# Penguin-jpg/clip-diffusion

Measured on NVIDIA B200. Metric: CLIP-guided cutouts/s fwd+bwd inside full guidance steps (= steps/s x cutouts per step) @512x512, higher is better.
Workload: dtype bf16

## Files before the change

clip_diffusion_b200/csrc/vit_attention_tc.cu:

```cuda
#include "common.cuh"
#include "tcgen05.cuh"

using namespace tc;

namespace {

constexpr int AT_THREADS = 512;
constexpr int MAX_BLK = 5;
static_assert((ATTN_TC_MAX_T + 63) / 64 <= MAX_BLK, "operand blocks of the longest sequence");
constexpr float LOG2E_F = 1.4426950408889634f;
constexpr uint32_t BLK_BYTES = 64 * 128;
constexpr uint32_t TILE_BYTES = 128 * 128;

__device__ __forceinline__ uint32_t pack_bf2(float a, float b) {
  __nv_bfloat162 v = __floats2bfloat162_rn(a, b);
  return *reinterpret_cast<uint32_t*>(&v);
}
__device__ __forceinline__ float ex2f(float x) {
  float y;
  asm("ex2.approx.ftz.f32 %0, %1;" : "=f"(y) : "f"(x));
  return y;
}
__device__ __forceinline__ float warp_max_f(float v) {
#pragma unroll
// ... 586 lines not shown
                w[j] = pack_bf2(p0, p1);
              }
            }
            lsum += a0 + a1;
            TRF(warp, g, 5 + hlf);
            if (!waited) { mbar_wait(bars.pfree(b), (use & 1u) ^ 1u); waited = true; }
            const uint32_t hb = sStage + b * TILE_BYTES + (uint32_t)rl * 128u;
            st_shared_v4(hb + (((uint32_t)(hlf * 64)) ^ sx), w[0], w[1], w[2], w[3]);
            st_shared_v4(hb + (((uint32_t)(hlf * 64 + 16)) ^ sx), w[4], w[5], w[6], w[7]);
            st_shared_v4(hb + (((uint32_t)(hlf * 64 + 32)) ^ sx), w[8], w[9], w[10], w[11]);
            st_shared_v4(hb + (((uint32_t)(hlf * 64 + 48)) ^ sx), w[12], w[13], w[14], w[15]);
          }
        }
        if (last_in_tile) {
          const int tp = tile & 1, a = 2 * wg + tp;
          const uint32_t u = tp ? wuse1 : wuse0;
          if (wvalid) {
            sm[(a * 4 + (int)(u & 3u)) * 128 + rl] = mref;
            sl[(a * 4 + (int)(u & 3u)) * 128 + rl] = lsum;
          }
          __syncwarp();
          if (lane == 0) mbar_arrive(bars.mready(a, u & 1u));
          if (tp) wuse1 = u + 1; else wuse0 = u + 1;
        }
        TRF(warp, g, 2);
        fence_proxy_async_smem();
        __syncwarp();
        if (lane == 0) mbar_arrive(bars.pready(b));
        TRF(warp, g, 3);
        blk += 2;
        while (blk >= nblk) { blk -= nblk; ++tile; }
      }
    }
  } else {
    const int q = warp & 3;
    const int rl = q * 32 + lane;
    const uint32_t t_lane = tmem_base + ((uint32_t)(q * 32) << 16);
    const float sl2 = p.scale * LOG2E_F;
    float* vedge2 = pvec + 808;
    uint32_t euse = 0;
    auto edge_a = [&](int wi, int eit, float& s0, float& s1) {
      const uint32_t opar = (uint32_t)eit & 1u;
      if (edge) {
        for (int b = 0; b < nblk_ld; ++b) { mbar_wait(bars.opk(b), opar); mbar_wait(bars.opq(b), opar); }
#ifdef CG_ATTN_TRACE
        long long* etr = (p.trace != nullptr && blockIdx.x == 0 && eit == 3) ? p.trace + ((warp * 64 + 60) << 3) : nullptr;
#else
        long long* etr = nullptr;
#endif
        const float2 se = fwd_edge_token_a(sQ, sK, Tp, sl2, pvec, etr);
        s0 = se.x;
        s1 = se.y;
      } else if (eit > 0) {
        mbar_wait(bars.qkfree(), (uint32_t)(eit - 1) & 1u);
      }
      __syncwarp();
      if (lane == 0) mbar_arrive(bars.qkfree());
    };
    auto edge_b = [&](int wi, int eit) {
      const int n = wi / heads, h = wi - n * heads, row0 = n * T, vb = eit & 1;
      if (edge) {
        for (int b = 0; b < nblk_ld; ++b) mbar_wait(bars.opv(vb, b), (uint32_t)(eit >> 1) & 1u);
#ifdef CG_ATTN_TRACE
        long long* etr = (p.trace != nullptr && blockIdx.x == 0 && eit == 3) ? p.trace + ((warp * 64 + 60) << 3) : nullptr;
#else
        long long* etr = nullptr;
#endif
        fwd_edge_token_b(sV0 + vb * opb, Tp, pvec, vedge2 + vb * 64, p.ctx + ((long long)(row0 + Tp)) * D + h * 64, p.lse + ((long long)n * heads + h) * T + Tp, etr);
      }
      __syncwarp();
      if (lane == 0) mbar_arrive(bars.vfree(vb));
    };
    float se0 = -INFINITY, se1 = -INFINITY, nse0 = -INFINITY, nse1 = -INFINITY;
    if ((int)blockIdx.x < nitems) { edge_a(blockIdx.x, 0, se0, se1); edge_b(blockIdx.x, 0); }
    int it = 0, gg0 = 0;
    for (int w = blockIdx.x; w < nitems; w += gridDim.x, ++it, gg0 += G) {
      const int n = w / heads, h = w - n * heads, row0 = n * T;
      const float* vedge = vedge2 + (it & 1) * 64;
      TRF(warp, 62, 0);
      TRI(warp, 0);
      for (int tile = 0; tile < ntiles; ++tile) {
        const int tp = tile & 1, a0 = tp, a1 = 2 + tp;
        const int ggt = gg0 + tile * nblk;
        const bool has0 = nblk > 1 || (ggt & 1) == 0, has1 = nblk > 1 || (ggt & 1) == 1;
        const uint32_t u0 = (euse >> (4 * a0)) & 15u, u1 = (euse >> (4 * a1)) & 15u;
        if (has0) { mbar_wait(bars.mready(a0, u0 & 1u), (u0 >> 1) & 1u); mbar_wait(bars.accfull(a0), u0 & 1u); }
        if (has1) { mbar_wait(bars.mready(a1, u1 & 1u), (u1 >> 1) & 1u); mbar_wait(bars.accfull(a1), u1 & 1u); }
        TRF(warp, tile, 0);
        tcgen05_fence_after();
        const int row = tile * 128 + rl;
        if (tile * 128 + q * 32 < Tp) {
          const float m0 = has0 ? sm[(a0 * 4 + (int)(u0 & 3u)) * 128 + rl] : -INFINITY, m1 = has1 ? sm[(a1 * 4 + (int)(u1 & 3u)) * 128 + rl] : -INFINITY;
          const float l0 = has0 ? sl[(a0 * 4 + (int)(u0 & 3u)) * 128 + rl] : 0.f, l1 = has1 ? sl[(a1 * 4 + (int)(u1 & 3u)) * 128 + rl] : 0.f;
          const float se = tile == 0 ? se0 : se1;
          const float M = fmaxf(fmaxf(m0, m1), se);
          const float f0 = has0 ? ex2f(m0 - M) : 0.f, f1 = has1 ? ex2f(m1 - M) : 0.f, fe = ex2f(se - M);
          const float L = l0 * f0 + l1 * f1 + fe;
          const float invL = __fdividef(1.f, L);
          const float g0 = f0 * invL, g1 = f1 * invL, ge = fe * invL;
          __nv_bfloat16* dst = p.ctx + ((long long)(row0 + row)) * D + h * 64;
#pragma unroll
          for (int c = 0; c < 64; c += 32) {
            uint32_t v0[32], v1[32], wv[16];
            if (has0) tmem_ld32(t_lane + 256u + (uint32_t)(a0 * 64 + c), v0);
            if (has1) tmem_ld32(t_lane + 256u + (uint32_t)(a1 * 64 + c), v1);
            tmem_ld_wait();
#pragma unroll
            for (int j = 0; j < 16; ++j) {
              float x0 = (has0 ? __uint_as_float(v0[2 * j]) * g0 : 0.f) + (has1 ? __uint_as_float(v1[2 * j]) * g1 : 0.f);
              float x1 = (has0 ? __uint_as_float(v0[2 * j + 1]) * g0 : 0.f) + (has1 ? __uint_as_float(v1[2 * j + 1]) * g1 : 0.f);
              if (edge) {
                const float2 ve = *reinterpret_cast<const float2*>(vedge + c + 2 * j);
                x0 = fmaf(ge, ve.x, x0);
                x1 = fmaf(ge, ve.y, x1);
              }
              wv[j] = pack_bf2(x0, x1);
            }
            if (row < Tp) { st256g(dst + c, wv); st256g(dst + c + 16, wv + 8); }
          }
          if (row < Tp) p.lse[((long long)n * heads + h) * T + row] = M * (1.f / LOG2E_F) + logf(L);
        }
        tcgen05_fence_before();
        __syncwarp();
        if (lane == 0) {
          if (has0) mbar_arrive(bars.accfree(a0));
          if (has1) mbar_arrive(bars.accfree(a1));
        }
        if (has0) euse = (euse & ~(15u << (4 * a0))) | (((u0 + 1u) & 15u) << (4 * a0));
        if (has1) euse = (euse & ~(15u << (4 * a1))) | (((u1 + 1u) & 15u) << (4 * a1));
        TRF(warp, tile, 1);
        if (tile == 0 && w + (int)gridDim.x < nitems) {
          TRF(warp, 61, 0);
          edge_a(w + gridDim.x, it + 1, nse0, nse1);
          edge_b(w + gridDim.x, it + 1);
          TRF(warp, 61, 1);
        }
      }
      se0 = nse0;
      se1 = nse1;
      TRF(warp, 62, 1);
      TRI(warp, 1);
    }
  }
  tcgen05_fence_before();
  __syncthreads();
  if (warp == 2) {
    tcgen05_fence_after();
    asm volatile("tcgen05.dealloc.cta_group::1.sync.aligned.b32 %0, %1;" ::"r"(tmem_base), "r"(512) : "memory");
  }
}

struct BBars {
  uint32_t base;
  __device__ __forceinline__ uint32_t sfull(int b) const { return base + 8u * b; }
  __device__ __forceinline__ uint32_t sfree(int b) const { return base + 24u + 8u * b; }
  __device__ __forceinline__ uint32_t pready(int pb) const { return base + 48u + 8u * pb; }
  __device__ __forceinline__ uint32_t pfree(int pb) const { return base + 64u + 8u * pb; }
  __device__ __forceinline__ uint32_t accfull(int a) const { return base + 80u + 8u * a; }
  __device__ __forceinline__ uint32_t accfree(int a) const { return base + 104u + 8u * a; }
  __device__ __forceinline__ uint32_t op(int o, int blk) const { return base + 128u + 8u * (o * MAX_BLK + blk); }
  __device__ __forceinline__ uint32_t opfree() const { return base + 288u; }
  __device__ __forceinline__ uint32_t cready(int par) const { return base + 296u + 8u * par; }
  __device__ __forceinline__ uint32_t tmem_slot() const { return base + 312u; }
};
constexpr uint32_t BBARS_BYTES = 320 + 16;
constexpr uint32_t BWD_FLOATS = 1280 + 1152 + 192 + 768;

#ifdef CG_ATTN_TRACE
#define TRB(slot, idx, ev) TRF(slot, idx, ev)
#else
#define TRB(slot, idx, ev) do { } while (0)
#endif

__device__ __forceinline__ void store_row64_bf16_axpy(__nv_bfloat16* dst, const uint32_t* a, const uint32_t* b, float coef, const float* vec) {
  uint32_t w[32];
#pragma unroll
  for (int j = 0; j < 16; ++j) {
    const float2 v0 = *reinterpret_cast<const float2*>(vec + 2 * j), v1 = *reinterpret_cast<const float2*>(vec + 32 + 2 * j);
    w[j] = pack_bf2(fmaf(coef, v0.x, __uint_as_float(a[2 * j])), fmaf(coef, v0.y, __uint_as_float(a[2 * j + 1])));
    w[16 + j] = pack_bf2(fmaf(coef, v1.x, __uint_as_float(b[2 * j])), fmaf(coef, v1.y, __uint_as_float(b[2 * j + 1])));
  }
#pragma unroll
  for (int j = 0; j < 4; ++j) st256g(dst + 16 * j, w + 8 * j);
}

__global__ void __launch_bounds__(AT_THREADS, 1)
    attn_bwd_tc_kernel(const __grid_constant__ CUtensorMap tmQKV, const __grid_constant__ CUtensorMap tmQKVtail, const __grid_constant__ CUtensorMap tmDO,
                       const __grid_constant__ CUtensorMap tmDOtail, const AttnParams p) {
  extern __shared__ __align__(1024) uint8_t smem_raw[];
  cg_griddep_launch();
  constexpr int NSB = 3;
  constexpr uint32_t STAGE_BYTES = 2 * TILE_BYTES;
  const int T = p.T, heads = p.heads, D = heads * 64;
  const int edge = p.edge, Tp = T - edge;
  const int warp = threadIdx.x >> 5, lane = threadIdx.x & 31;
  const int ntiles = p.ntiles, nblk = p.nblk, nblk_ld = p.nblk_ld;
  const int per_phase = ntiles * nblk, G = 2 * per_phase, nitems = p.nitems;
  const uint32_t opb = (uint32_t)((nblk_ld - 1) * 64 + p.ld_tail) * 128u;
  const uint32_t base = (smem_u32(smem_raw) + 1023u) & ~1023u;
  const uint32_t sOp0 = base;
  const uint32_t sStage = base + 4 * opb;
  const uint32_t sF = sStage + 2 * STAGE_BYTES;
  float* fscr = reinterpret_cast<float*>(smem_raw + (sF - smem_u32(smem_raw)));
  float* csts = fscr;
  float* ev = fscr + 1280;
  float* evec = fscr + 2432;
  float* epart = fscr + 2624;
  BBars bars{sF + BWD_FLOATS * 4};

  if (warp == 0 && lane == 0) {
    asm volatile("prefetch.tensormap [%0];" ::"l"(&tmQKV) : "memory");
    asm volatile("prefetch.tensormap [%0];" ::"l"(&tmQKVtail) : "memory");
    asm volatile("prefetch.tensormap [%0];" ::"l"(&tmDO) : "memory");
    asm volatile("prefetch.tensormap [%0];" ::"l"(&tmDOtail) : "memory");
    for (int b = 0; b < 3; ++b) {
      mbar_init(bars.sfull(b), 2); mbar_init(bars.sfree(b), 4);
      mbar_init(bars.accfull(b), 2); mbar_init(bars.accfree(b), 4);
    }
    for (int b = 0; b < 2; ++b) { mbar_init(bars.pready(b), 4); mbar_init(bars.pfree(b), 2); mbar_init(bars.cready(b), 4); }
    for (int o = 0; o < 4; ++o)
      for (int k = 0; k < MAX_BLK; ++k) mbar_init(bars.op(o, k), 1);
    mbar_init(bars.opfree(), 8);
    asm volatile("fence.mbarrier_init.release.cluster;" ::: "memory");
  }
  if (warp == 2) {
    asm volatile("tcgen05.alloc.cta_group::1.sync.aligned.shared::cta.b32 [%0], %1;" ::"r"(bars.tmem_slot()), "r"(512) : "memory");
    asm volatile("tcgen05.relinquish_alloc_permit.cta_group::1.sync.aligned;" ::: "memory");
  }
  cg_griddep_wait();
  tcgen05_fence_before();
  __syncthreads();
  tcgen05_fence_after();
  uint32_t tmem_base;
  asm volatile("ld.shared.b32 %0, [%1];" : "=r"(tmem_base) : "r"(bars.tmem_slot()) : "memory");

  if (warp < 4) {
    const uint32_t elected = elect_one();
    const uint32_t id_full = idesc_bf16(64, false), id_tail = idesc_bf16(p.tail_rows, false), id_acc = idesc_bf16(64, true);
    uint32_t cuse = 0;
    int it = 0, gg0 = 0;
    for (int w = blockIdx.x; w < nitems; w += gridDim.x, ++it, gg0 += G) {
      const uint32_t opar = (uint32_t)it & 1u;
      uint32_t loaded = 0;
      auto need = [&](int o, int blk) {
        const uint32_t bit = 1u << (o * MAX_BLK + blk);
        if (!(loaded & bit)) { mbar_wait(bars.op(o, blk), opar); loaded |= bit; }
      };
      if (warp == 3) {
        if (elected) {
          if (it > 0) mbar_wait(bars.opfree(), (uint32_t)(it - 1) & 1u);
          const int n = w / heads, h = w - n * heads, row0 = n * T;
          auto load = [&](int o, int blk) {
            const bool tail = blk == nblk_ld - 1;
            const uint32_t bar = bars.op(o, blk);
            mbar_arrive_expect_tx(bar, (uint32_t)(tail ? p.ld_tail : 64) * 128u);
            if (o < 3) tma_load_2d(sOp0 + o * opb + blk * BLK_BYTES, tail ? &tmQKVtail : &tmQKV, bar, o * D + h * 64, row0 + blk * 64);
            else tma_load_2d(sOp0 + o * opb + blk * BLK_BYTES, tail ? &tmDOtail : &tmDO, bar, h * 64, row0 + blk * 64);
          };
          const int first = nblk_ld < 2 ? nblk_ld : 2;
          load(1, 0);
#pragma unroll 1
          for (int k = 0; k < first; ++k) load(0, k);
          load(2, 0);
#pragma unroll 1
          for (int k = 0; k < first; ++k) load(3, k);
#pragma unroll 1
          for (int k = 1; k < nblk_ld; ++k) { load(1, k); load(2, k); }
#pragma unroll 1
          for (int k = first; k < nblk_ld; ++k) { load(0, k); load(3, k); }
          if (w + (int)gridDim.x < nitems) {
            const int w2 = w + gridDim.x, n2 = w2 / heads, h2 = w2 - n2 * heads;
#pragma unroll 1
            for (int k = 0; k < nblk_ld; ++k) {
              const bool tail = k == nblk_ld - 1;
#pragma unroll 1
              for (int o = 0; o < 3; ++o) tma_prefetch_2d(tail ? &tmQKVtail : &tmQKV, o * D + h2 * 64, n2 * T + k * 64);
              tma_prefetch_2d(tail ? &tmDOtail : &tmDO, h2 * 64, n2 * T + k * 64);
            }
          }
        }
        __syncwarp();
      }
      int phase = 0, tile = 0, blk = 0;
      if (warp < 2) {
        for (int g = 0; g < G; ++g) {
          const int gg = gg0 + g, b = gg % NSB;
          const bool transposed = phase == 1;
          const int oa = warp == 0 ? (transposed ? 1 : 0) : (transposed ? 2 : 3);
          const int ob = warp == 0 ? (transposed ? 0 : 1) : (transposed ? 3 : 2);
          need(oa, 2 * tile);
          if (2 * tile + 1 < nblk) need(oa, 2 * tile + 1);
          need(ob, blk);
          mbar_wait(bars.sfree(b), ((uint32_t)(gg / NSB) & 1u) ^ 1u);
          TRB(warp, g, 0);
          tcgen05_fence_after();
          const uint32_t d_s = tmem_base + (uint32_t)(b * 128) + (warp == 1 ? 64u : 0u);
          const uint64_t ad = make_smem_desc(sOp0 + oa * opb + tile * TILE_BYTES), bd = make_smem_desc(sOp0 + ob * opb + blk * BLK_BYTES);
          const uint32_t idesc = blk == nblk - 1 ? id_tail : id_full;
          if (elected) {
#pragma unroll
            for (int k = 0; k < 4; ++k) umma_bf16(d_s, ad + (uint64_t)(2 * k), bd + (uint64_t)(2 * k), idesc, k != 0 ? 1u : 0u);
            umma_commit(bars.sfull(b));
          }
          __syncwarp();
          TRB(warp, g, 1);
          if (++blk == nblk) { blk = 0; if (++tile == ntiles) { tile = 0; ++phase; } }
        }
      } else {
        const int wi = warp - 2;
        for (int g = 0; g < G; ++g) {
          const int gg = gg0 + g, pb = gg & 1;
          const int a = phase == 1 ? 2 : (tile & 1);
          const bool does_mma = phase == 1 || wi == 0;
          const int ob = phase == 0 ? 1 : (wi == 0 ? 3 : 0);
          if (does_mma) need(ob, blk);
          mbar_wait(bars.pready(pb), (uint32_t)(gg >> 1) & 1u);
          TRB(warp, g, 0);
          if (blk == 0) {
            if (phase == 1) {
              mbar_wait(bars.accfree(2), ((cuse >> 2) & 1u) ^ 1u);
              if (tile == 0) { mbar_wait(bars.accfree(0), (cuse & 1u) ^ 1u); mbar_wait(bars.accfree(1), ((cuse >> 1) & 1u) ^ 1u); }
            } else {
              mbar_wait(bars.accfree(a), ((cuse >> a) & 1u) ^ 1u);
              mbar_wait(bars.accfree(2), ((cuse >> 2) & 1u) ^ 1u);
            }
          }
          tcgen05_fence_after();
          const int ksteps = (blk == nblk - 1 ? p.tail_rows : 64) >> 4;
          const uint32_t stage = sStage + pb * STAGE_BYTES + (wi == 1 ? TILE_BYTES : 0u);
          const uint32_t d_acc = tmem_base + (a == 2 ? 384u : 384u + 64u * a) + (wi == 1 ? 64u : 0u);
          const uint64_t ad = make_smem_desc(stage), bd = make_smem_desc(sOp0 + ob * opb + blk * BLK_BYTES);
          const bool last = blk == nblk - 1;
          if (elected) {
            if (does_mma) {
              for (int k = 0; k < ksteps; ++k) umma_bf16(d_acc, ad + (uint64_t)(2 * k), bd + (uint64_t)(128 * k), id_acc, (blk | k) != 0 ? 1u : 0u);
              umma_commit(bars.pfree(pb));
              if (last) umma_commit(bars.accfull(a));
            } else {
              mbar_arrive(bars.pfree(pb));
              if (last) mbar_arrive(bars.accfull(a));
            }
          }
          __syncwarp();
          TRB(warp, g, 1);
          if (last) cuse ^= 1u << a;
          if (++blk == nblk) { blk = 0; if (++tile == ntiles) { tile = 0; ++phase; } }
        }
      }
#pragma unroll 1
      for (int o = 0; o < 4; ++o)
#pragma unroll 1
        for (int k = 0; k < nblk_ld; ++k) need(o, k);
      if (elected) umma_commit(bars.opfree());
      __syncwarp();
    }
  } else if (warp < 12) {
    const int wg = (warp - 4) >> 2;
    const int q = warp & 3;
    const int rl = q * 32 + lane;
    const uint32_t t_lane = tmem_base + ((uint32_t)(q * 32) << 16);
    const float scale = p.scale, sl2 = p.scale * LOG2E_F;
    const int tail_cols = Tp - (nblk - 1) * 64, tail_cols16 = p.tail_rows;
    const uint32_t sx = (uint32_t)(rl & 7) << 4;
    int it = 0, gg0 = 0;
    for (int w = blockIdx.x; w < nitems; w += gridDim.x, ++it, gg0 += G) {
      mbar_wait(bars.cready(it & 1), (uint32_t)(it >> 1) & 1u);
      const float* cst = csts + (it & 1) * 640;
      float rc0 = 0.f, rc1 = 0.f;
      int phase = 0, tile = 0, blk = wg, cur_tile = -1;
      while (blk >= nblk) { blk -= nblk; if (++tile == ntiles) { tile = 0; ++phase; } }
      for (int g = wg; g < G; g += 2) {
        const int gg = gg0 + g;
        if (phase == 0 && tile != cur_tile) {
          const int row = tile * 128 + rl;
          rc0 = row < Tp ? cst[row] : 0.f;
          rc1 = row < Tp ? cst[320 + row] : 0.f;
          cur_tile = tile;
        }
        const bool wvalid = tile * 128 + q * 32 < Tp;
        const bool tail = blk == nblk - 1;
        const int ncols = tail ? tail_cols : 64, ncols16 = tail ? tail_cols16 : 64;
        const int b = gg % NSB, pb = gg & 1;
        const uint32_t suse = (uint32_t)(gg / NSB), puse = (uint32_t)(gg >> 1);
        TRB(warp, g, 0);
        mbar_wait(bars.sfull(b), suse & 1u);
        TRB(warp, g, 1);
        tcgen05_fence_after();
        const uint32_t t_s = t_lane + (uint32_t)(b * 128);
        const uint32_t stage = sStage + pb * STAGE_BYTES + (uint32_t)rl * 128u;
        if (!wvalid) {
          tcgen05_fence_before();
          __syncwarp();
          if (lane == 0) mbar_arrive(bars.sfree(b));
          mbar_wait(bars.pfree(pb), (puse & 1u) ^ 1u);
        } else {
          uint32_t sv[2][16], dv[2][16], w0[8], w1[8];
          const int npieces = ncols16 >> 4;
          tmem_ld16(t_s, sv[0]);
          tmem_ld16(t_s + 64u, dv[0]);
          tmem_ld_wait();
          bool waited = false;
#pragma unroll
          for (int pc = 0; pc < 4; ++pc) {
            if (pc < npieces) {
              const int cur = pc & 1;
              if (pc + 1 < npieces) {
                tmem_ld16(t_s + (uint32_t)(16 * (pc + 1)), sv[cur ^ 1]);
                tmem_ld16(t_s + 64u + (uint32_t)(16 * (pc + 1)), dv[cur ^ 1]);
              }
              if (phase == 0) {
#pragma unroll
                for (int j = 0; j < 8; ++j) {
                  float p0 = ex2f(fmaf(__uint_as_float(sv[cur][2 * j]), sl2, rc0)), p1 = ex2f(fmaf(__uint_as_float(sv[cur][2 * j + 1]), sl2, rc0));
                  if (tail) { if (16 * pc + 2 * j >= ncols) p0 = 0.f; if (16 * pc + 2 * j + 1 >= ncols) p1 = 0.f; }
                  w0[j] = pack_bf2(p0 * fmaf(__uint_as_float(dv[cur][2 * j]), scale, rc1), p1 * fmaf(__uint_as_float(dv[cur][2 * j + 1]), scale, rc1));
                }
              } else {
                const float* nl = cst + blk * 64 + 16 * pc;
                const float* dl = nl + 320;
#pragma unroll
                for (int j = 0; j < 8; ++j) {
                  const float2 l2 = *reinterpret_cast<const float2*>(nl + 2 * j), d2 = *reinterpret_cast<const float2*>(dl + 2 * j);
                  float p0 = ex2f(fmaf(__uint_as_float(sv[cur][2 * j]), sl2, l2.x)), p1 = ex2f(fmaf(__uint_as_float(sv[cur][2 * j + 1]), sl2, l2.y));
                  if (tail) { if (16 * pc + 2 * j >= ncols) p0 = 0.f; if (16 * pc + 2 * j + 1 >= ncols) p1 = 0.f; }
                  w0[j] = pack_bf2(p0, p1);
                  w1[j] = pack_bf2(p0 * fmaf(__uint_as_float(dv[cur][2 * j]), scale, d2.x), p1 * fmaf(__uint_as_float(dv[cur][2 * j + 1]), scale, d2.y));
                }
              }
              if (!waited) { mbar_wait(bars.pfree(pb), (puse & 1u) ^ 1u); waited = true; }
              {
                const uint32_t c0 = ((uint32_t)(pc * 32)) ^ sx, c1 = ((uint32_t)(pc * 32 + 16)) ^ sx;
                st_shared_v4(stage + c0, w0[0], w0[1], w0[2], w0[3]);
                st_shared_v4(stage + c1, w0[4], w0[5], w0[6], w0[7]);
                if (phase == 1) {
                  st_shared_v4(stage + TILE_BYTES + c0, w1[0], w1[1], w1[2], w1[3]);
                  st_shared_v4(stage + TILE_BYTES + c1, w1[4], w1[5], w1[6], w1[7]);
                }
              }
              if (pc + 1 < npieces) {
                tmem_ld_wait();
              } else {
                tcgen05_fence_before();
                __syncwarp();
                if (lane == 0) mbar_arrive(bars.sfree(b));
              }
            }
          }
        }
        TRB(warp, g, 2);
        fence_proxy_async_smem();
        __syncwarp();
        if (lane == 0) mbar_arrive(bars.pready(pb));
        TRB(warp, g, 3);
        blk += 2;
        while (blk >= nblk) { blk -= nblk; if (++tile == ntiles) { tile = 0; ++phase; } }
      }
    }
  } else {
    const int q = warp & 3;
    const int rl = q * 32 + lane;
    const uint32_t t_lane = tmem_base + ((uint32_t)(q * 32) << 16);
    const float scale = p.scale, sl2 = p.scale * LOG2E_F;
    uint32_t euse = 0;
    auto load_consts = [&](int item, int par) {
      const int n = item / heads, h = item - n * heads;
      const float* lb = p.lse + ((long long)n * heads + h) * T;
      const __nv_bfloat16* ob = p.ctx_in + ((long long)n * T) * D + h * 64;
      const __nv_bfloat16* gb = p.dctx_in + ((long long)n * T) * D + h * 64;
      float* c = csts + par * 640;
      for (int i = rl; i < 320; i += 128) {
        float dl = 0.f, nl = -INFINITY;
        if (i < T) {
          const uint4* o4 = reinterpret_cast<const uint4*>(ob + (long long)i * D);
          const uint4* g4 = reinterpret_cast<const uint4*>(gb + (long long)i * D);
          uint4 xo[8], xg[8];
#pragma unroll
          for (int k = 0; k < 8; ++k) { xo[k] = __ldg(o4 + k); xg[k] = __ldg(g4 + k); }
          float d0 = 0.f, d1 = 0.f;
#pragma unroll
          for (int k = 0; k < 8; k += 2) { d0 = dot8p(xo[k], xg[k], d0); d1 = dot8p(xo[k + 1], xg[k + 1], d1); }
          dl = d0 + d1;
          nl = -lb[i] * LOG2E_F;
        }
        c[i] = nl;
        c[320 + i] = -p.scale * dl;
      }
      __syncwarp();
      if (lane == 0) mbar_arrive(bars.cready(par));
    };
    if ((int)blockIdx.x < nitems) load_consts(blockIdx.x, 0);
    int it = 0;
    for (int w = blockIdx.x; w < nitems; w += gridDim.x, ++it) {
      const int n = w / heads, h = w - n * heads, row0 = n * T;
      const uint32_t opar = (uint32_t)it & 1u;
      if (w + (int)gridDim.x < nitems) load_consts(w + gridDim.x, (it + 1) & 1);
      const float* cst = csts + (it & 1) * 640;
      __nv_bfloat16* out = p.dqkv + ((long long)row0) * 3 * D + h * 64;
      TRB(warp, 62, 0);
      TRI(warp, 0);
      if (edge) {
        for (int o = 0; o < 4; ++o)
          for (int k = 0; k < nblk_ld; ++k) mbar_wait(bars.op(o, k), opar);
        mbar_wait(bars.cready(it & 1), (uint32_t)(it >> 1) & 1u);
        TRB(warp, 61, 0);
        const uint32_t sQ = sOp0, sK = sOp0 + opb, sV = sOp0 + 2 * opb, sDO = sOp0 + 3 * opb;
        const float nle = cst[Tp], dle = cst[320 + Tp];
        const int g = lane >> 2, t = lane & 3;
        {
          uint32_t vbk[8], vbv[8], vbq[8], vbd[8];
          load_vec_bfrag(sK, Tp, vbk);
          load_vec_bfrag(sV, Tp, vbv);
          load_vec_bfrag(sQ, Tp, vbq);
          load_vec_bfrag(sDO, Tp, vbd);
#pragma unroll 1
          for (int rg = q; rg < (Tp >> 4); rg += 4) {
            const float2 s_c = mv16(sQ, rg * 16, vbk), dp_c = mv16(sDO, rg * 16, vbv), s_r = mv16(sK, rg * 16, vbq), dp_r = mv16(sV, rg * 16, vbd);
            if (t == 0) {
#pragma unroll
              for (int hh = 0; hh < 2; ++hh) {
                const int i = rg * 16 + g + 8 * hh;
                const float p_c = ex2f(fmaf(hh ? s_c.y : s_c.x, sl2, cst[i]));
                ev[i] = p_c;
                ev[288 + i] = p_c * fmaf(hh ? dp_c.y : dp_c.x, scale, cst[320 + i]);
                const float p_r = ex2f(fmaf(hh ? s_r.y : s_r.x, sl2, nle));
                ev[576 + i] = p_r;
                ev[864 + i] = p_r * fmaf(hh ? dp_r.y : dp_r.x, scale, dle);
              }
            }
          }
        }
        {
          const uint32_t eo = (uint32_t)Tp * 128u + (uint32_t)lane * 4u;
          const uint32_t wq = lds32(sQ + eo), wk = lds32(sK + eo), wv = lds32(sV + eo), wd = lds32(sDO + eo);
          const float s_e = warp_sum(fmaf(bf_lo(wq), bf_lo(wk), bf_hi(wq) * bf_hi(wk)));
          const float dp_e = warp_sum(fmaf(bf_lo(wd), bf_lo(wv), bf_hi(wd) * bf_hi(wv)));
          const float p_e = ex2f(fmaf(s_e, sl2, nle)), ds_e = p_e * fmaf(dp_e, scale, dle);
          if (rl == 0) { ev[Tp] = p_e; ev[288 + Tp] = ds_e; ev[576 + Tp] = p_e; ev[864 + Tp] = ds_e; }
          if (rl >= 1 && rl < 16) { ev[Tp + rl] = 0.f; ev[288 + Tp + rl] = 0.f; ev[576 + Tp + rl] = 0.f; ev[864 + Tp + rl] = 0.f; }
          if (q == 0) {
            evec[2 * lane] = bf_lo(wk); evec[2 * lane + 1] = bf_hi(wk);
            evec[64 + 2 * lane] = bf_lo(wq); evec[64 + 2 * lane + 1] = bf_hi(wq);
            evec[128 + 2 * lane] = bf_lo(wd); evec[128 + 2 * lane + 1] = bf_hi(wd);
          }
        }
        asm volatile("bar.sync 2, 128;" ::: "memory");
        {
          const int ngrp = (Tp >> 4) + 1;
#pragma unroll 1
          for (int pr = 0; pr < 3; ++pr) {
            const uint32_t buf = pr == 0 ? sK : (pr == 1 ? sQ : sDO);
            const float* vec = ev + (pr == 0 ? 864 : (pr == 1 ? 288 : 0));
            float acc[8][4];
#pragma unroll
            for (int nn = 0; nn < 8; ++nn) acc[nn][0] = acc[nn][1] = acc[nn][2] = acc[nn][3] = 0.f;
#pragma unroll 1
            for (int ks = q; ks < ngrp; ks += 4) vm16(buf, ks * 16, vec, acc);
            if (lane < 4) {
#pragma unroll
              for (int nn = 0; nn < 8; ++nn) *reinterpret_cast<float2*>(epart + (pr * 4 + q) * 64 + 8 * nn + 2 * t) = make_float2(acc[nn][0], acc[nn][1]);
            }
          }
          asm volatile("bar.sync 2, 128;" ::: "memory");
          if (q < 3) {
            const float* pp = epart + q * 256 + 2 * lane;
            const float2 x0 = *reinterpret_cast<const float2*>(pp), x1 = *reinterpret_cast<const float2*>(pp + 64);
            const float2 x2 = *reinterpret_cast<const float2*>(pp + 128), x3 = *reinterpret_cast<const float2*>(pp + 192);
            reinterpret_cast<uint32_t*>(out + (long long)Tp * 3 * D + q * D)[lane] = pack_bf2((x0.x + x1.x) + (x2.x + x3.x), (x0.y + x1.y) + (x2.y + x3.y));
          }
        }
        TRB(warp, 61, 1);
      }
      __syncwarp();
      if (lane == 0) mbar_arrive(bars.opfree());
      for (int tc = 0; tc < 2 * ntiles; ++tc) {
        const int phase = tc >= ntiles ? 1 : 0, tile = tc - phase * ntiles;
        const int a = phase == 1 ? 2 : (tile & 1);
        const int row = tile * 128 + rl;
        mbar_wait(bars.accfull(a), (euse >> a) & 1u);
        TRB(warp, tc, 0);
        tcgen05_fence_after();
        if (tile * 128 + q * 32 < Tp) {
          uint32_t v0[32], v1[32];
          const uint32_t col = a == 2 ? 384u : 384u + 64u * a;
          tmem_ld32(t_lane + col, v0);
          tmem_ld32(t_lane + col + 32u, v1);
          tmem_ld_wait();
          __nv_bfloat16* orow = out + (long long)row * 3 * D;
          if (phase == 0) {
            if (row < Tp) {
              if (edge) store_row64_bf16_axpy(orow, v0, v1, ev[288 + row], evec);
              else store_row64_bf16(orow, v0, v1, 1.f);
            }
          } else {
            if (row < Tp) {
              if (edge) store_row64_bf16_axpy(orow + 2 * D, v0, v1, ev[576 + row], evec + 128);
              else store_row64_bf16(orow + 2 * D, v0, v1, 1.f);
            }
            tmem_ld32(t_lane + col + 64u, v0);
            tmem_ld32(t_lane + col + 96u, v1);
            tmem_ld_wait();
            if (row < Tp) {
              if (edge) store_row64_bf16_axpy(orow + D, v0, v1, ev[864 + row], evec + 64);
              else store_row64_bf16(orow + D, v0, v1, 1.f);
            }
          }
        }
        tcgen05_fence_before();
        __syncwarp();
        if (lane == 0) mbar_arrive(bars.accfree(a));
        euse ^= 1u << a;
        TRB(warp, tc, 1);
      }
      TRB(warp, 62, 1);
      TRI(warp, 1);
    }
  }
  tcgen05_fence_before();
  __syncthreads();
  if (warp == 2) {
    tcgen05_fence_after();
    asm volatile("tcgen05.dealloc.cta_group::1.sync.aligned.b32 %0, %1;" ::"r"(tmem_base), "r"(512) : "memory");
  }
}

long long* g_trace = nullptr;

void set_geometry(AttnParams& p, int T, int heads, bool causal) {
  p.T = T; p.heads = heads; p.scale = 0.125f;
  p.trace = g_trace;
  p.edge = (!causal && T > 1 && (T - 1) % 64 == 0) ? 1 : 0;
  const int Tp = T - p.edge;
  p.ntiles = (Tp + 127) / 128;
  p.nblk = (Tp + 63) / 64;
  p.tail_rows = ((Tp - (p.nblk - 1) * 64) + 15) & ~15;
  p.nblk_ld = p.nblk + p.edge;
  p.ld_tail = p.edge ? 16 : p.tail_rows;
}

int make_operand_maps(CUtensorMap& full, CUtensorMap& tail, const void* ptr, long long rows, long long cols, const AttnParams& p) {
  const int rc = cg_make_tensor_map_bf16(&full, ptr, rows, cols, cols, 64);
  return rc ? rc : cg_make_tensor_map_bf16(&tail, ptr, rows, cols, cols, p.ld_tail);
}

template <auto kernel, typename... Maps>
int launch_persistent(AttnParams& p, int Nimg, size_t extra, cudaStream_t s, const Maps&... maps) {
  const size_t opb = (size_t)((p.nblk_ld - 1) * 64 + p.ld_tail) * 128;
  const size_t smem = 1024 + 4 * opb + 4 * (size_t)TILE_BYTES + extra;
  p.nitems = Nimg * p.heads;
  const int grid = p.nitems < cg_num_sms() ? p.nitems : cg_num_sms();
  static size_t configured[CG_MAX_DEVICES] = {};
  const int dev = cg_device_index();
  if (smem > configured[dev]) {
    CG_CUDA(cudaFuncSetAttribute(kernel, cudaFuncAttributeMaxDynamicSharedMemorySize, (int)smem));
    configured[dev] = smem;
  }
  CG_CUDA(cg_launch_pdl(kernel, dim3(grid), dim3(AT_THREADS), smem, s, maps..., p));
  return 0;
}

template <bool CAUSAL>
int launch_attn_fwd_tc(const void* qkv, int Nimg, int T, int heads, void* ctx, float* lse, cudaStream_t s) {
  AttnParams p = {};
  p.ctx = reinterpret_cast<__nv_bfloat16*>(ctx);
  p.lse = lse;
  set_geometry(p, T, heads, CAUSAL);
  CUtensorMap tq, tqt;
  const int rc = make_operand_maps(tq, tqt, qkv, (long long)Nimg * T, 3LL * heads * 64, p);
  if (rc) return rc;
  return launch_persistent<attn_fwd_tc_kernel<CAUSAL>>(p, Nimg, FWD_FLOATS * 4 + FBARS_BYTES, s, tq, tqt);
}

}

int cg_attention_fwd_tc(const void* qkv, int Nimg, int T, int heads, void* ctx, float* lse, cudaStream_t s) {
  return launch_attn_fwd_tc<false>(qkv, Nimg, T, heads, ctx, lse, s);
}

extern "C" int cg_attention_causal_fwd(const void* qkv, int Nseq, int T, int heads, void* ctx, float* lse, void* stream) {
  CG_REQUIRE(qkv && ctx && lse && Nseq > 0 && T > 0 && heads > 0, "cg_attention_causal_fwd: bad arguments");
  CG_REQUIRE(T <= ATTN_TC_MAX_T, "cg_attention_causal_fwd: T=%d exceeds the tcgen05 kernel's limit (%d)", T, ATTN_TC_MAX_T);
  return launch_attn_fwd_tc<true>(qkv, Nseq, T, heads, ctx, lse, cg_stream(stream));
}

int cg_attention_bwd_tc(const void* qkv, const void* ctx, const void* dctx, const float* lse, int Nimg, int T, int heads, void* dqkv, cudaStream_t s) {
  AttnParams p = {};
  p.lse = const_cast<float*>(lse);
  p.ctx_in = reinterpret_cast<const __nv_bfloat16*>(ctx);
  p.dctx_in = reinterpret_cast<const __nv_bfloat16*>(dctx);
  p.dqkv = reinterpret_cast<__nv_bfloat16*>(dqkv);
  set_geometry(p, T, heads, false);
  const int D = heads * 64;
  CUtensorMap tq, tqt, td, tdt;
  int rc = make_operand_maps(tq, tqt, qkv, (long long)Nimg * T, 3LL * D, p);
  if (!rc) rc = make_operand_maps(td, tdt, dctx, (long long)Nimg * T, D, p);
  if (rc) return rc;
  return launch_persistent<attn_bwd_tc_kernel>(p, Nimg, BWD_FLOATS * 4 + BBARS_BYTES, s, tq, tqt, td, tdt);
}

extern "C" void cg_debug_attention_trace(void* buf) { g_trace = reinterpret_cast<long long*>(buf); }
```

Measured before the change: 1357.

## Restructure attention backward into a single pass with per-tile dK/dV and fused dQ

The backward attention kernel drops its two-phase schedule, where the softmax gradient tiles were recomputed a second time in transposed form for dQ. It now makes one pass per key tile: dK/dV accumulate into dedicated TMEM columns, and dQ is accumulated by the dK MMA warp from the same staged dS tiles, with a zig-zag query-block order that lets paired stages be consumed together. It also reorders the TMA loads, prefetches the next item's context and LSE into L2, and moves the edge-row work and constant loads to overlap with the first epilogue tile. This roughly halves the S/dP MMA and exp work, at the cost of more complex barrier protocols and fewer score buffers when there are more than two tiles.

```diff
diff --git a/clip_diffusion_b200/csrc/vit_attention_tc.cu b/clip_diffusion_b200/csrc/vit_attention_tc.cu
--- a/clip_diffusion_b200/csrc/vit_attention_tc.cu
+++ b/clip_diffusion_b200/csrc/vit_attention_tc.cu
@@ -762,18 +762,20 @@
 
 struct BBars {
   uint32_t base;
-  __device__ __forceinline__ uint32_t sfull(int b) const { return base + 8u * b; }
-  __device__ __forceinline__ uint32_t sfree(int b) const { return base + 24u + 8u * b; }
-  __device__ __forceinline__ uint32_t pready(int pb) const { return base + 48u + 8u * pb; }
-  __device__ __forceinline__ uint32_t pfree(int pb) const { return base + 64u + 8u * pb; }
-  __device__ __forceinline__ uint32_t accfull(int a) const { return base + 80u + 8u * a; }
-  __device__ __forceinline__ uint32_t accfree(int a) const { return base + 104u + 8u * a; }
-  __device__ __forceinline__ uint32_t op(int o, int blk) const { return base + 128u + 8u * (o * MAX_BLK + blk); }
-  __device__ __forceinline__ uint32_t opfree() const { return base + 288u; }
-  __device__ __forceinline__ uint32_t cready(int par) const { return base + 296u + 8u * par; }
-  __device__ __forceinline__ uint32_t tmem_slot() const { return base + 312u; }
+  __device__ __forceinline__ uint32_t sfull(int wg) const { return base + 8u * wg; }
+  __device__ __forceinline__ uint32_t sfree(int wg) const { return base + 16u + 8u * wg; }
+  __device__ __forceinline__ uint32_t pready(int pb) const { return base + 32u + 8u * pb; }
+  __device__ __forceinline__ uint32_t pfree(int pb) const { return base + 48u + 8u * pb; }
+  __device__ __forceinline__ uint32_t kvfull() const { return base + 64u; }
+  __device__ __forceinline__ uint32_t kvfree() const { return base + 72u; }
+  __device__ __forceinline__ uint32_t dqfull() const { return base + 80u; }
+  __device__ __forceinline__ uint32_t dqfree() const { return base + 88u; }
+  __device__ __forceinline__ uint32_t op(int o, int blk) const { return base + 96u + 8u * (o * MAX_BLK + blk); }
+  __device__ __forceinline__ uint32_t opfree() const { return base + 256u; }
+  __device__ __forceinline__ uint32_t cready(int par) const { return base + 264u + 8u * par; }
+  __device__ __forceinline__ uint32_t tmem_slot() const { return base + 280u; }
 };
-constexpr uint32_t BBARS_BYTES = 320 + 16;
+constexpr uint32_t BBARS_BYTES = 288 + 16;
 constexpr uint32_t BWD_FLOATS = 1280 + 1152 + 192 + 768;
 
 #ifdef CG_ATTN_TRACE
@@ -794,18 +796,21 @@
   for (int j = 0; j < 4; ++j) st256g(dst + 16 * j, w + 8 * j);
 }
 
+__device__ __forceinline__ int bwd_qblk(int pos, int start_odd, int nblk) { return start_odd ? (pos == 0 ? nblk - 1 : pos - 1) : pos; }
+__device__ __forceinline__ uint32_t bwd_dq_col(int m) { return m < 2 ? 384u + 64u * (uint32_t)m : 128u; }
+
 __global__ void __launch_bounds__(AT_THREADS, 1)
     attn_bwd_tc_kernel(const __grid_constant__ CUtensorMap tmQKV, const __grid_constant__ CUtensorMap tmQKVtail, const __grid_constant__ CUtensorMap tmDO,
                        const __grid_constant__ CUtensorMap tmDOtail, const AttnParams p) {
   extern __shared__ __align__(1024) uint8_t smem_raw[];
   cg_griddep_launch();
-  constexpr int NSB = 3;
   constexpr uint32_t STAGE_BYTES = 2 * TILE_BYTES;
   const int T = p.T, heads = p.heads, D = heads * 64;
   const int edge = p.edge, Tp = T - edge;
   const int warp = threadIdx.x >> 5, lane = threadIdx.x & 31;
   const int ntiles = p.ntiles, nblk = p.nblk, nblk_ld = p.nblk_ld;
-  const int per_phase = ntiles * nblk, G = 2 * per_phase, nitems = p.nitems;
+  const int G = ntiles * nblk, nitems = p.nitems;
+  const int nsb = ntiles > 2 ? 1 : 2;
   const uint32_t opb = (uint32_t)((nblk_ld - 1) * 64 + p.ld_tail) * 128u;
   const uint32_t base = (smem_u32(smem_raw) + 1023u) & ~1023u;
   const uint32_t sOp0 = base;
@@ -823,11 +828,12 @@
     asm volatile("prefetch.tensormap [%0];" ::"l"(&tmQKVtail) : "memory");
     asm volatile("prefetch.tensormap [%0];" ::"l"(&tmDO) : "memory");
     asm volatile("prefetch.tensormap [%0];" ::"l"(&tmDOtail) : "memory");
-    for (int b = 0; b < 3; ++b) {
+    for (int b = 0; b < 2; ++b) {
       mbar_init(bars.sfull(b), 2); mbar_init(bars.sfree(b), 4);
-      mbar_init(bars.accfull(b), 2); mbar_init(bars.accfree(b), 4);
+      mbar_init(bars.pready(b), 4); mbar_init(bars.pfree(b), 2); mbar_init(bars.cready(b), 4);
     }
-    for (int b = 0; b < 2; ++b) { mbar_init(bars.pready(b), 4); mbar_init(bars.pfree(b), 2); mbar_init(bars.cready(b), 4); }
+    mbar_init(bars.kvfull(), 2); mbar_init(bars.kvfree(), 4);
+    mbar_init(bars.dqfull(), 1); mbar_init(bars.dqfree(), 4);
     for (int o = 0; o < 4; ++o)
       for (int k = 0; k < MAX_BLK; ++k) mbar_init(bars.op(o, k), 1);
     mbar_init(bars.opfree(), 8);
@@ -847,7 +853,9 @@
   if (warp < 4) {
     const uint32_t elected = elect_one();
     const uint32_t id_full = idesc_bf16(64, false), id_tail = idesc_bf16(p.tail_rows, false), id_acc = idesc_bf16(64, true);
-    uint32_t cuse = 0;
+    const uint32_t id_dq = id_acc | (1u << 15);
+    const int dq_ks_last = (Tp - (ntiles - 1) * 128 + 15) >> 4;
+    uint32_t kvuse = 0, dquse = 0;
     int it = 0, gg0 = 0;
     for (int w = blockIdx.x; w < nitems; w += gridDim.x, ++it, gg0 += G) {
       const uint32_t opar = (uint32_t)it & 1u;
@@ -868,16 +876,16 @@
             else tma_load_2d(sOp0 + o * opb + blk * BLK_BYTES, tail ? &tmDOtail : &tmDO, bar, h * 64, row0 + blk * 64);
           };
           const int first = nblk_ld < 2 ? nblk_ld : 2;
-          load(1, 0);
-#pragma unroll 1
-          for (int k = 0; k < first; ++k) load(0, k);
-          load(2, 0);
-#pragma unroll 1
-          for (int k = 0; k < first; ++k) load(3, k);
-#pragma unroll 1
-          for (int k = 1; k < nblk_ld; ++k) { load(1, k); load(2, k); }
-#pragma unroll 1
-          for (int k = first; k < nblk_ld; ++k) { load(0, k); load(3, k); }
+#pragma unroll 1
+          for (int k = 0; k < first; ++k) load(1, k);
+          load(0, 0);
+#pragma unroll 1
+          for (int k = 0; k < first; ++k) load(2, k);
+          load(3, 0);
+#pragma unroll 1
+          for (int k = 1; k < nblk_ld; ++k) { load(0, k); load(3, k); }
+#pragma unroll 1
+          for (int k = first; k < nblk_ld; ++k) { load(1, k); load(2, k); }
           if (w + (int)gridDim.x < nitems) {
             const int w2 = w + gridDim.x, n2 = w2 / heads, h2 = w2 - n2 * heads;
 #pragma unroll 1
@@ -890,72 +898,81 @@
           }
         }
         __syncwarp();
-      }
-      int phase = 0, tile = 0, blk = 0;
+        if (w + (int)gridDim.x < nitems) {
+          const int w2 = w + gridDim.x, n2 = w2 / heads, h2 = w2 - n2 * heads;
+          const __nv_bfloat16* ob = p.ctx_in + ((long long)n2 * T) * D + h2 * 64;
+#pragma unroll 1
+          for (int i = lane; i < T; i += 32) asm volatile("prefetch.global.L2 [%0];" ::"l"(ob + (long long)i * D));
+          if (32 * lane < T) asm volatile("prefetch.global.L2 [%0];" ::"l"(p.lse + ((long long)n2 * heads + h2) * T + 32 * lane));
+        }
+      }
+      int t = 0, pos = 0;
       if (warp < 2) {
+        const int oa = warp == 0 ? 1 : 2, ob = warp == 0 ? 0 : 3;
         for (int g = 0; g < G; ++g) {
-          const int gg = gg0 + g, b = gg % NSB;
-          const bool transposed = phase == 1;
-          const int oa = warp == 0 ? (transposed ? 1 : 0) : (transposed ? 2 : 3);
-          const int ob = warp == 0 ? (transposed ? 0 : 1) : (transposed ? 3 : 2);
-          need(oa, 2 * tile);
-          if (2 * tile + 1 < nblk) need(oa, 2 * tile + 1);
-          need(ob, blk);
-          mbar_wait(bars.sfree(b), ((uint32_t)(gg / NSB) & 1u) ^ 1u);
+          const int gg = gg0 + g;
+          const int j = bwd_qblk(pos, (gg0 + t * nblk) & 1, nblk);
+          need(oa, 2 * t);
+          if (2 * t + 1 < nblk) need(oa, 2 * t + 1);
+          need(ob, j);
+          if (gg >= nsb) mbar_wait(bars.sfree((gg - nsb) & 1), (uint32_t)((gg - nsb) >> 1) & 1u);
           TRB(warp, g, 0);
           tcgen05_fence_after();
-          const uint32_t d_s = tmem_base + (uint32_t)(b * 128) + (warp == 1 ? 64u : 0u);
-          const uint64_t ad = make_smem_desc(sOp0 + oa * opb + tile * TILE_BYTES), bd = make_smem_desc(sOp0 + ob * opb + blk * BLK_BYTES);
-          const uint32_t idesc = blk == nblk - 1 ? id_tail : id_full;
+          const uint32_t d_s = tmem_base + (uint32_t)((gg % nsb) * 128) + (warp == 1 ? 64u : 0u);
+          const uint64_t ad = make_smem_desc(sOp0 + oa * opb + t * TILE_BYTES), bd = make_smem_desc(sOp0 + ob * opb + j * BLK_BYTES);
+          const uint32_t idesc = j == nblk - 1 ? id_tail : id_full;
           if (elected) {
 #pragma unroll
             for (int k = 0; k < 4; ++k) umma_bf16(d_s, ad + (uint64_t)(2 * k), bd + (uint64_t)(2 * k), idesc, k != 0 ? 1u : 0u);
-            umma_commit(bars.sfull(b));
+            umma_commit(bars.sfull(gg & 1));
           }
           __syncwarp();
           TRB(warp, g, 1);
-          if (++blk == nblk) { blk = 0; if (++tile == ntiles) { tile = 0; ++phase; } }
+          if (++pos == nblk) { pos = 0; ++t; }
         }
       } else {
-        const int wi = warp - 2;
+        const bool is_dk = warp == 3;
+        bool dq_waited = false;
         for (int g = 0; g < G; ++g) {
           const int gg = gg0 + g, pb = gg & 1;
-          const int a = phase == 1 ? 2 : (tile & 1);
-          const bool does_mma = phase == 1 || wi == 0;
-          const int ob = phase == 0 ? 1 : (wi == 0 ? 3 : 0);
-          if (does_mma) need(ob, blk);
+          const int j = bwd_qblk(pos, (gg0 + t * nblk) & 1, nblk);
+          const bool last_pos = pos == nblk - 1, last = last_pos && t == ntiles - 1;
+          const bool dq_now = is_dk && ((j & 1) || j == nblk - 1);
+          need(is_dk ? 0 : 3, j);
+          if (dq_now) { need(1, 2 * t); if (2 * t + 1 < nblk) need(1, 2 * t + 1); }
           mbar_wait(bars.pready(pb), (uint32_t)(gg >> 1) & 1u);
           TRB(warp, g, 0);
-          if (blk == 0) {
-            if (phase == 1) {
-              mbar_wait(bars.accfree(2), ((cuse >> 2) & 1u) ^ 1u);
-              if (tile == 0) { mbar_wait(bars.accfree(0), (cuse & 1u) ^ 1u); mbar_wait(bars.accfree(1), ((cuse >> 1) & 1u) ^ 1u); }
-            } else {
-              mbar_wait(bars.accfree(a), ((cuse >> a) & 1u) ^ 1u);
-              mbar_wait(bars.accfree(2), ((cuse >> 2) & 1u) ^ 1u);
+          if (pos == 0) mbar_wait(bars.kvfree(), (kvuse & 1u) ^ 1u);
+          if (dq_now && !dq_waited) { mbar_wait(bars.dqfree(), (dquse & 1u) ^ 1u); dq_waited = true; }
+          tcgen05_fence_after();
+          const int ksteps = (j == nblk - 1 ? p.tail_rows : 64) >> 4;
+          const uint32_t stage = sStage + pb * STAGE_BYTES;
+          const uint32_t d_acc = tmem_base + (is_dk ? 320u : 256u);
+          const uint64_t ad = make_smem_desc(stage + (is_dk ? 0u : TILE_BYTES)), bd = make_smem_desc(sOp0 + (is_dk ? 0 : 3) * opb + j * BLK_BYTES);
+          if (elected) {
+            for (int k = 0; k < ksteps; ++k) umma_bf16(d_acc, ad + (uint64_t)(2 * k), bd + (uint64_t)(128 * k), id_acc, (pos | k) != 0 ? 1u : 0u);
+            if (dq_now) {
+              const bool paired = (j & 1) != 0;
+              uint64_t aq = make_smem_desc(paired ? sStage : stage);
+              aq = (aq & ~((uint64_t)0x3FFF << 16)) | ((uint64_t)((paired ? STAGE_BYTES : TILE_BYTES) >> 4) << 16);
+              const uint64_t bq = make_smem_desc(sOp0 + opb + t * TILE_BYTES);
+              const uint32_t d_dq = tmem_base + bwd_dq_col(j >> 1);
+              const int kq = t == ntiles - 1 ? dq_ks_last : 8;
+              for (int k = 0; k < kq; ++k) umma_bf16(d_dq, aq + (uint64_t)(128 * k), bq + (uint64_t)(128 * k), id_dq, (t | k) != 0 ? 1u : 0u);
+              if (paired) umma_commit(bars.pfree(0));
+              umma_commit(bars.pfree(pb));
+            } else if (!is_dk) {
+              umma_commit(bars.pfree(pb));
             }
-          }
-          tcgen05_fence_after();
-          const int ksteps = (blk == nblk - 1 ? p.tail_rows : 64) >> 4;
-          const uint32_t stage = sStage + pb * STAGE_BYTES + (wi == 1 ? TILE_BYTES : 0u);
-          const uint32_t d_acc = tmem_base + (a == 2 ? 384u : 384u + 64u * a) + (wi == 1 ? 64u : 0u);
-          const uint64_t ad = make_smem_desc(stage), bd = make_smem_desc(sOp0 + ob * opb + blk * BLK_BYTES);
-          const bool last = blk == nblk - 1;
-          if (elected) {
-            if (does_mma) {
-              for (int k = 0; k < ksteps; ++k) umma_bf16(d_acc, ad + (uint64_t)(2 * k), bd + (uint64_t)(128 * k), id_acc, (blk | k) != 0 ? 1u : 0u);
-              umma_commit(bars.pfree(pb));
-              if (last) umma_commit(bars.accfull(a));
-            } else {
-              mbar_arrive(bars.pfree(pb));
-              if (last) mbar_arrive(bars.accfull(a));
-            }
+            if (last_pos) umma_commit(bars.kvfull());
+            if (is_dk && last) umma_commit(bars.dqfull());
           }
           __syncwarp();
           TRB(warp, g, 1);
-          if (last) cuse ^= 1u << a;
-          if (++blk == nblk) { blk = 0; if (++tile == ntiles) { tile = 0; ++phase; } }
-        }
+          if (last_pos) ++kvuse;
+          if (++pos == nblk) { pos = 0; ++t; }
+        }
+        if (is_dk) ++dquse;
       }
 #pragma unroll 1
       for (int o = 0; o < 4; ++o)
@@ -976,32 +993,27 @@
     for (int w = blockIdx.x; w < nitems; w += gridDim.x, ++it, gg0 += G) {
       mbar_wait(bars.cready(it & 1), (uint32_t)(it >> 1) & 1u);
       const float* cst = csts + (it & 1) * 640;
-      float rc0 = 0.f, rc1 = 0.f;
-      int phase = 0, tile = 0, blk = wg, cur_tile = -1;
-      while (blk >= nblk) { blk -= nblk; if (++tile == ntiles) { tile = 0; ++phase; } }
-      for (int g = wg; g < G; g += 2) {
+      int g = (wg ^ gg0) & 1, t = 0, pos = g;
+      if (pos >= nblk) { pos -= nblk; ++t; }
+      for (; g < G; g += 2) {
         const int gg = gg0 + g;
-        if (phase == 0 && tile != cur_tile) {
-          const int row = tile * 128 + rl;
-          rc0 = row < Tp ? cst[row] : 0.f;
-          rc1 = row < Tp ? cst[320 + row] : 0.f;
-          cur_tile = tile;
-        }
-        const bool wvalid = tile * 128 + q * 32 < Tp;
-        const bool tail = blk == nblk - 1;
+        const int j = bwd_qblk(pos, (gg0 + t * nblk) & 1, nblk);
+        const bool wvalid = t * 128 + q * 32 < Tp;
+        const bool rvalid = t * 128 + rl < Tp;
+        const bool tail = j == nblk - 1;
         const int ncols = tail ? tail_cols : 64, ncols16 = tail ? tail_cols16 : 64;
-        const int b = gg % NSB, pb = gg & 1;
-        const uint32_t suse = (uint32_t)(gg / NSB), puse = (uint32_t)(gg >> 1);
+        const int pb = gg & 1;
+        const uint32_t puse = (uint32_t)(gg >> 1);
         TRB(warp, g, 0);
-        mbar_wait(bars.sfull(b), suse & 1u);
+        mbar_wait(bars.sfull(wg), puse & 1u);
         TRB(warp, g, 1);
         tcgen05_fence_after();
-        const uint32_t t_s = t_lane + (uint32_t)(b * 128);
+        const uint32_t t_s = t_lane + (uint32_t)((gg % nsb) * 128);
         const uint32_t stage = sStage + pb * STAGE_BYTES + (uint32_t)rl * 128u;
         if (!wvalid) {
           tcgen05_fence_before();
           __syncwarp();
-          if (lane == 0) mbar_arrive(bars.sfree(b));
+          if (lane == 0) mbar_arrive(bars.sfree(wg));
           mbar_wait(bars.pfree(pb), (puse & 1u) ^ 1u);
         } else {
           uint32_t sv[2][16], dv[2][16], w0[8], w1[8];
@@ -1018,41 +1030,30 @@
                 tmem_ld16(t_s + (uint32_t)(16 * (pc + 1)), sv[cur ^ 1]);
                 tmem_ld16(t_s + 64u + (uint32_t)(16 * (pc + 1)), dv[cur ^ 1]);
               }
-              if (phase == 0) {
-#pragma unroll
-                for (int j = 0; j < 8; ++j) {
-                  float p0 = ex2f(fmaf(__uint_as_float(sv[cur][2 * j]), sl2, rc0)), p1 = ex2f(fmaf(__uint_as_float(sv[cur][2 * j + 1]), sl2, rc0));
-                  if (tail) { if (16 * pc + 2 * j >= ncols) p0 = 0.f; if (16 * pc + 2 * j + 1 >= ncols) p1 = 0.f; }
-                  w0[j] = pack_bf2(p0 * fmaf(__uint_as_float(dv[cur][2 * j]), scale, rc1), p1 * fmaf(__uint_as_float(dv[cur][2 * j + 1]), scale, rc1));
-                }
-              } else {
-                const float* nl = cst + blk * 64 + 16 * pc;
-                const float* dl = nl + 320;
-#pragma unroll
-                for (int j = 0; j < 8; ++j) {
-                  const float2 l2 = *reinterpret_cast<const float2*>(nl + 2 * j), d2 = *reinterpret_cast<const float2*>(dl + 2 * j);
-                  float p0 = ex2f(fmaf(__uint_as_float(sv[cur][2 * j]), sl2, l2.x)), p1 = ex2f(fmaf(__uint_as_float(sv[cur][2 * j + 1]), sl2, l2.y));
-                  if (tail) { if (16 * pc + 2 * j >= ncols) p0 = 0.f; if (16 * pc + 2 * j + 1 >= ncols) p1 = 0.f; }
-                  w0[j] = pack_bf2(p0, p1);
-                  w1[j] = pack_bf2(p0 * fmaf(__uint_as_float(dv[cur][2 * j]), scale, d2.x), p1 * fmaf(__uint_as_float(dv[cur][2 * j + 1]), scale, d2.y));
-                }
+              const float* nl = cst + j * 64 + 16 * pc;
+              const float* dl = nl + 320;
+#pragma unroll
+              for (int jj = 0; jj < 8; ++jj) {
+                const float2 l2 = *reinterpret_cast<const float2*>(nl + 2 * jj), d2 = *reinterpret_cast<const float2*>(dl + 2 * jj);
+                float p0 = ex2f(fmaf(__uint_as_float(sv[cur][2 * jj]), sl2, l2.x)), p1 = ex2f(fmaf(__uint_as_float(sv[cur][2 * jj + 1]), sl2, l2.y));
+                if (tail) { if (16 * pc + 2 * jj >= ncols) p0 = 0.f; if (16 * pc + 2 * jj + 1 >= ncols) p1 = 0.f; }
+                w0[jj] = pack_bf2(p0, p1);
+                w1[jj] = rvalid ? pack_bf2(p0 * fmaf(__uint_as_float(dv[cur][2 * jj]), scale, d2.x), p1 * fmaf(__uint_as_float(dv[cur][2 * jj + 1]), scale, d2.y)) : 0u;
               }
               if (!waited) { mbar_wait(bars.pfree(pb), (puse & 1u) ^ 1u); waited = true; }
               {
                 const uint32_t c0 = ((uint32_t)(pc * 32)) ^ sx, c1 = ((uint32_t)(pc * 32 + 16)) ^ sx;
-                st_shared_v4(stage + c0, w0[0], w0[1], w0[2], w0[3]);
-                st_shared_v4(stage + c1, w0[4], w0[5], w0[6], w0[7]);
-                if (phase == 1) {
-                  st_shared_v4(stage + TILE_BYTES + c0, w1[0], w1[1], w1[2], w1[3]);
-                  st_shared_v4(stage + TILE_BYTES + c1, w1[4], w1[5], w1[6], w1[7]);
-                }
+                st_shared_v4(stage + c0, w1[0], w1[1], w1[2], w1[3]);
+                st_shared_v4(stage + c1, w1[4], w1[5], w1[6], w1[7]);
+                st_shared_v4(stage + TILE_BYTES + c0, w0[0], w0[1], w0[2], w0[3]);
+                st_shared_v4(stage + TILE_BYTES + c1, w0[4], w0[5], w0[6], w0[7]);
               }
               if (pc + 1 < npieces) {
                 tmem_ld_wait();
               } else {
                 tcgen05_fence_before();
                 __syncwarp();
-                if (lane == 0) mbar_arrive(bars.sfree(b));
+                if (lane == 0) mbar_arrive(bars.sfree(wg));
               }
             }
           }
@@ -1062,8 +1063,8 @@
         __syncwarp();
         if (lane == 0) mbar_arrive(bars.pready(pb));
         TRB(warp, g, 3);
-        blk += 2;
-        while (blk >= nblk) { blk -= nblk; if (++tile == ntiles) { tile = 0; ++phase; } }
+        pos += 2;
+        while (pos >= nblk) { pos -= nblk; ++t; }
       }
     }
   } else {
@@ -1071,7 +1072,7 @@
     const int rl = q * 32 + lane;
     const uint32_t t_lane = tmem_base + ((uint32_t)(q * 32) << 16);
     const float scale = p.scale, sl2 = p.scale * LOG2E_F;
-    uint32_t euse = 0;
+    uint32_t kvu = 0, dqu = 0;
     auto load_consts = [&](int item, int par) {
       const int n = item / heads, h = item - n * heads;
       const float* lb = p.lse + ((long long)n * heads + h) * T;
@@ -1099,11 +1100,12 @@
       if (lane == 0) mbar_arrive(bars.cready(par));
     };
     if ((int)blockIdx.x < nitems) load_consts(blockIdx.x, 0);
+    const bool single_tile = ntiles == 1;
     int it = 0;
     for (int w = blockIdx.x; w < nitems; w += gridDim.x, ++it) {
       const int n = w / heads, h = w - n * heads, row0 = n * T;
       const uint32_t opar = (uint32_t)it & 1u;
-      if (w + (int)gridDim.x < nitems) load_consts(w + gridDim.x, (it + 1) & 1);
+      if (single_tile && w + (int)gridDim.x < nitems) load_consts(w + gridDim.x, (it + 1) & 1);
       const float* cst = csts + (it & 1) * 640;
       __nv_bfloat16* out = p.dqkv + ((long long)row0) * 3 * D + h * 64;
       TRB(warp, 62, 0);
@@ -1112,6 +1114,7 @@
         for (int o = 0; o < 4; ++o)
           for (int k = 0; k < nblk_ld; ++k) mbar_wait(bars.op(o, k), opar);
         mbar_wait(bars.cready(it & 1), (uint32_t)(it >> 1) & 1u);
+        asm volatile("bar.sync 2, 128;" ::: "memory");
         TRB(warp, 61, 0);
         const uint32_t sQ = sOp0, sK = sOp0 + opb, sV = sOp0 + 2 * opb, sDO = sOp0 + 3 * opb;
         const float nle = cst[Tp], dle = cst[320 + Tp];
@@ -1154,7 +1157,13 @@
           }
         }
         asm volatile("bar.sync 2, 128;" ::: "memory");
-        {
+        TRB(warp, 61, 1);
+      }
+      auto edge_rows_and_release = [&]() {
+        if (edge) {
+          TRB(warp, 60, 0);
+          const uint32_t sQ = sOp0, sK = sOp0 + opb, sDO = sOp0 + 3 * opb;
+          const int t = lane & 3;
           const int ngrp = (Tp >> 4) + 1;
 #pragma unroll 1
           for (int pr = 0; pr < 3; ++pr) {
@@ -1177,26 +1186,28 @@
             const float2 x2 = *reinterpret_cast<const float2*>(pp + 128), x3 = *reinterpret_cast<const float2*>(pp + 192);
             reinterpret_cast<uint32_t*>(out + (long long)Tp * 3 * D + q * D)[lane] = pack_bf2((x0.x + x1.x) + (x2.x + x3.x), (x0.y + x1.y) + (x2.y + x3.y));
           }
-        }
-        TRB(warp, 61, 1);
-      }
-      __syncwarp();
-      if (lane == 0) mbar_arrive(bars.opfree());
+          TRB(warp, 60, 1);
+        }
+        __syncwarp();
+        if (lane == 0) mbar_arrive(bars.opfree());
+      };
+      if (single_tile) edge_rows_and_release();
       for (int tc = 0; tc < 2 * ntiles; ++tc) {
-        const int phase = tc >= ntiles ? 1 : 0, tile = tc - phase * ntiles;
-        const int a = phase == 1 ? 2 : (tile & 1);
+        const bool is_dq = tc >= ntiles;
+        const int tile = is_dq ? tc - ntiles : tc;
         const int row = tile * 128 + rl;
-        mbar_wait(bars.accfull(a), (euse >> a) & 1u);
-        TRB(warp, tc, 0);
+        if (!is_dq) mbar_wait(bars.kvfull(), kvu & 1u);
+        else if (tile == 0) mbar_wait(bars.dqfull(), dqu & 1u);
+        TRB(warp, is_dq ? 4 + tile : tile, 0);
         tcgen05_fence_after();
         if (tile * 128 + q * 32 < Tp) {
           uint32_t v0[32], v1[32];
-          const uint32_t col = a == 2 ? 384u : 384u + 64u * a;
+          const uint32_t col = is_dq ? bwd_dq_col(tile) : 256u;
           tmem_ld32(t_lane + col, v0);
           tmem_ld32(t_lane + col + 32u, v1);
           tmem_ld_wait();
           __nv_bfloat16* orow = out + (long long)row * 3 * D;
-          if (phase == 0) {
+          if (is_dq) {
             if (row < Tp) {
               if (edge) store_row64_bf16_axpy(orow, v0, v1, ev[288 + row], evec);
               else store_row64_bf16(orow, v0, v1, 1.f);
@@ -1215,11 +1226,17 @@
             }
           }
         }
-        tcgen05_fence_before();
-        __syncwarp();
-        if (lane == 0) mbar_arrive(bars.accfree(a));
-        euse ^= 1u << a;
-        TRB(warp, tc, 1);
+        if (!is_dq || tile == ntiles - 1) {
+          tcgen05_fence_before();
+          __syncwarp();
+          if (lane == 0) mbar_arrive(is_dq ? bars.dqfree() : bars.kvfree());
+          if (is_dq) ++dqu; else ++kvu;
+        }
+        TRB(warp, is_dq ? 4 + tile : tile, 1);
+        if (tc == 0 && !single_tile) {
+          edge_rows_and_release();
+          if (w + (int)gridDim.x < nitems) load_consts(w + gridDim.x, (it + 1) & 1);
+        }
       }
       TRB(warp, 62, 1);
       TRI(warp, 1);
```

After: 1378 (median of 6 runs). 1.02x the previous value.
